# KentaYoshii/Raymarcher

Measured on AMD Instinct MI355X. Metric: Mpixels/s at 3840x2160 Mandelbulb, 256 march steps, higher is better.
Workload: dtype f32

## Files before the change

raymarcher_amd/csrc/rm_device.hip.h:

```cpp
#pragma once
#include "../../include/raymarcher_amd.h"
#include <type_traits>

#include "rm_math.hip.h"
#include "rm_internal.h"

namespace rm {

struct V3 { float x, y, z; };
struct V4 { float x, y, z, w; };

RM_DEV V3 v3(float x, float y, float z) { return V3{x, y, z}; }
RM_DEV V4 v4(float x, float y, float z, float w) { return V4{x, y, z, w}; }
RM_DEV V3 add(V3 a, V3 b) { return v3(a.x + b.x, a.y + b.y, a.z + b.z); }
RM_DEV V3 sub(V3 a, V3 b) { return v3(a.x - b.x, a.y - b.y, a.z - b.z); }
RM_DEV V3 mul(V3 a, V3 b) { return v3(a.x * b.x, a.y * b.y, a.z * b.z); }
RM_DEV V3 scale(V3 a, float s) { return v3(a.x * s, a.y * s, a.z * s); }
RM_DEV V3 neg(V3 a) { return v3(-a.x, -a.y, -a.z); }
RM_DEV V3 madd(V3 a, float s, V3 b) { return v3(fma(a.x, s, b.x), fma(a.y, s, b.y), fma(a.z, s, b.z)); }
RM_DEV float dot2(float ax, float ay, float bx, float by) { return fma(ay, by, ax * bx); }
RM_DEV float dot(V3 a, V3 b) { return fma(a.z, b.z, fma(a.y, b.y, a.x * b.x)); }
RM_DEV float len2(float x, float y) { return sqrt_(dot2(x, y, x, y)); }
RM_DEV float len(V3 a) { return sqrt_(dot(a, a)); }
RM_DEV V3 normalize(V3 a) { float inv = rcp_(len(a)); return scale(a, inv); }
// ... 6 lines not shown
  return (k < 0.0f) ? v3(0.0f, 0.0f, 0.0f) : r;
}
RM_DEV V3 mix(V3 a, V3 b, float t) { return v3(mix_(a.x, b.x, t), mix_(a.y, b.y, t), mix_(a.z, b.z, t)); }

constexpr float kSurfaceDist = 0.001f;

struct Counters { unsigned long long evals, iters, shades, fbm9, fbmd8, shapes; };

}
#include "rm_scene_block.h"
#include "rm_sampler.hip.h"
#include "rm_env.hip.h"
namespace rm {

struct LightSplit { int part; float *slot; int tileIndex; };
struct SceneMin { int idx; float d; V4 trap; };
struct MarchRes { int obj; float d; V4 trap; };
struct Hit { V3 rd, p, n; int obj; };
struct RenderOut { V3 col; int isEnv; float d; };


RM_DEV float sdBox(V3 p, float bx, float by, float bz) {
  float qx = fabs_(p.x) - bx, qy = fabs_(p.y) - by, qz = fabs_(p.z) - bz;
  V3 qm = v3(max_(qx, 0.0f), max_(qy, 0.0f), max_(qz, 0.0f));
  return len(qm) + min_(max_(qx, max_(qy, qz)), 0.0f);
}
RM_DEV float sdCone(V3 p, float r, float h) {
  float pox = len2(p.x, p.z) - r, poy = p.y + h;
  float ex = -r, ey = 2.0f * h;
  float t = clamp_(RM_DIVR_CONST(dot2(pox, poy, ex, ey), dot2(ex, ey, ex, ey)), 0.0f, 1.0f);
  float qx = fma(-ex, t, pox), qy = fma(-ey, t, poy);
  float d = len2(qx, qy);
  return (max_(qx, qy) > 0.0f) ? d : -min_(d, poy);
}
RM_DEV float sdCylinder(V3 p, float h, float r) {
  float dx = len2(p.x, p.z) - r, dy = fabs_(p.y) - h;
  return min_(max_(dx, dy), 0.0f) + len2(max_(dx, 0.0f), max_(dy, 0.0f));
}
RM_DEV float sdOctahedron(V3 p, float s) {
  p = v3(fabs_(p.x), fabs_(p.y), fabs_(p.z));
  float m = ((p.x + p.y) + p.z) - s;
  float rx = fma(3.0f, p.x, -m), ry = fma(3.0f, p.y, -m), rz = fma(3.0f, p.z, -m);
  bool cx = rx < 0.0f, cy = ry < 0.0f, cz = rz < 0.0f;
  V3 q = cx ? p : (cy ? v3(p.y, p.z, p.x) : v3(p.z, p.x, p.y));
  float k = clamp_(0.5f * ((q.z - q.y) + s), 0.0f, s);
  float dl = len(v3(q.x, (q.y - s) + k, q.z - k));
  return (cx || cy || cz) ? dl : (m * 0.57735027f);
}
RM_DEV float sdTorus(V3 p, float tx, float ty) { return len2(len2(p.x, p.z) - tx, p.y) - ty; }
RM_DEV float sdCapsule(V3 p, float h, float r) {
  p.y = p.y - clamp_(p.y, 0.0f, h);
  return len(p) - r;
}
RM_DEV float sdDeathStar(V3 p2, float ra, float rb, float d) {
  float px = p2.x, py = len2(p2.y, p2.z);
  float a = (((ra * ra) - (rb * rb)) + (d * d)) / (2.0f * d);
  float b = sqrt_(max_((ra * ra) - (a * a), 0.0f));
  float inner = len2(px - a, py - b);
  float outer = max_(len2(px, py) - ra, -(len2(px - d, py) - rb));
  return (fma(px, b, -(py * a)) > d * max_(b - py, 0.0f)) ? inner : outer;
}

RM_DEV float sdMandelBrot(const SceneBlock *sb, float px, float py) {
  float ltime = fma(-0.5f, cos_(sb->g.iTime * 0.06f), 0.5f);
  float zoom = pow_(0.9f, 50.0f * ltime);
  float k = (0.045f * zoom) * fma(-ltime, 0.5f, 1.0f);
  float cx = -0.745f - k, cy = 0.186f - k;
  float ld2 = 1.0f;
  float lz2 = dot2(px, py, px, py);
  const int n = sb->s.maxSteps;
  for (int i = 0; i < n; i++) {
    ld2 = ld2 * (4.0f * lz2);
    float nx = fma(px, px, -(py * py)) + cx;
    float ny = fma(2.0f * px, py, cy);
    px = nx; py = ny;
    lz2 = dot2(px, py, px, py);
    if (lz2 > 200.0f) break;
  }
  float d = sqrt_(lz2 / ld2) * log_(lz2);
  return sqrt_(clamp_((150.0f / zoom) * d, 0.0f, 1.0f));
}

enum BulbMode { BULB_GENERIC = 0, BULB_TRIG8 = 1, BULB_ALGEBRAIC8 = 2 };
template <int COUNT, int MODE, bool TRAPMIN, bool TRAP, bool NOJULIA = false>
RM_DEV float bulbIterate(const SceneBlock *sb, V3 pos, V4 &resColor, Counters &cnt) {
  const float power = (MODE == BULB_GENERIC) ? sb->g.power : 8.0f;
  const float pexp = (power - 1.0f) / 2.0f;
  const int iters = sb->s.fractalIters;
  const bool julia = !NOJULIA && len2(sb->g.juliaSeed[0], sb->g.juliaSeed[1]) != 0.0f;
  const bool angleSafe = (MODE != BULB_GENERIC) || fabs_(power) < 1.0e6f;
  const PowPlan planPower = powPlanUniform(power), planPexp = powPlanUniform(pexp);
  V3 w = pos;
  float m = dot(w, w);
  V4 trap = v4(fabs_(w.x), fabs_(w.y), fabs_(w.z), m);
  float dz = 1.0f;
  const V3 c = NOJULIA ? pos : (julia ? v3(sb->g.juliaSeed[0], sb->g.juliaSeed[1], 0.0f) : pos);
  for (int i = 0; i < iters; i++) {
    if (COUNT) cnt.iters++;
    const float mx = absmax_(w.x, w.z);
    const bool raw = (MODE != BULB_ALGEBRAIC8) && __ballot(!(mx >= 3.5527136788e-15f) || !(m < __builtin_inff())) == 0;
    auto step = [&](auto rawTag) __attribute__((always_inline)) {
      constexpr bool RAW = decltype(rawTag)::value;
      float r = RAW ? sqrt_noscale_(m) : sqrt_fast_(m);
      if (MODE == BULB_ALGEBRAIC8) {
        dz = fma(8.0f * (((m * m) * m) * r), dz, 1.0f);
        float rho = sqrt_fast_(dot2(w.x, w.z, w.x, w.z));
        float inv = rcp_(rho);
        float cz = (rho == 0.0f) ? 1.0f : w.z * inv, sx = (rho == 0.0f) ? 0.0f : w.x * inv;
        float re = w.y, im = rho;
#pragma unroll
        for (int k = 0; k < 3; k++) {
          float t = fma(re, re, -(im * im));
          im = 2.0f * (re * im);
          re = t;
          t = fma(cz, cz, -(sx * sx));
          sx = 2.0f * (cz * sx);
          cz = t;
        }
        w = v3(fma(im, sx, c.x), re + c.y, fma(im, cz, c.z));
      } else {
        float pm, pr;
        if (MODE == BULB_TRIG8) {
          pm = (m * (m * m)) * r;
          float r2 = r * r, r4 = r2 * r2;
          pr = r4 * r4;
        } else {
          pm = powApply(m, pexp, planPexp);
          pr = powApply(r, power, planPower);
        }
        dz = fma(power * pm, dz, 1.0f);
        float b = power * acos_(RAW ? w.y * rcp_raw_(r) : divr_(w.y, r));
        float a = power * atan2_mx_<RAW>(w.x, w.z, mx);
        float sb_, cb_, sa_, ca_;
        if (angleSafe) { sincos_inrange_(b, sb_, cb_); sincos_inrange_(a, sa_, ca_); }
        else { sincos_(b, sb_, cb_); sincos_(a, sa_, ca_); }
        w = v3(fma(pr, sb_ * sa_, c.x), fma(pr, cb_, c.y), fma(pr, sb_ * ca_, c.z));
      }
    };
    if (raw) step(std::true_type{}); else step(std::false_type{});
    if (TRAP) {
      if (TRAPMIN) trap = v4(trap.x, hwmin_abs_(trap.y, w.y), hwmin_abs_(trap.z, w.z), hwmin_(trap.w, m));
      else trap = v4(trap.x, min_(trap.y, fabs_(w.y)), min_(trap.z, fabs_(w.z)), min_(trap.w, m));
    }
    m = dot(w, w);
    if (m > 2.0f) break;
  }
  resColor = v4(m, trap.y, trap.z, trap.w);
  return divr_((0.25f * log_(m)) * sqrt_fast_(m), dz);
}
template <int COUNT, bool TRAPMIN, bool TRAP, bool PLAIN = false>
RM_DEV float sdMandelBulb(const SceneBlock *sb, V3 pos, V4 &resColor, Counters &cnt) {
  if (PLAIN || sb->g.power == 8.0f) {
    if (sb->s.features & RM_FEAT_BULB_POWER8_ALGEBRAIC) return bulbIterate<COUNT, BULB_ALGEBRAIC8, TRAPMIN, TRAP, PLAIN>(sb, pos, resColor, cnt);
    return bulbIterate<COUNT, BULB_TRIG8, TRAPMIN, TRAP, PLAIN>(sb, pos, resColor, cnt);
  }
  return bulbIterate<COUNT, BULB_GENERIC, TRAPMIN, TRAP>(sb, pos, resColor, cnt);
}

RM_DEV float sdSierpinski(V3 p) {
  const float Scale = 1.85f, Offset = 2.0f;
  const float k = Offset * (Scale - 1.0f);
  for (int n = 0; n < 14; n++) {
    if (p.x + p.y < 0.0f) { float t = p.x; p.x = -p.y; p.y = -t; }
    if (p.x + p.z < 0.0f) { float t = p.x; p.x = -p.z; p.z = -t; }
    if (p.y + p.z < 0.0f) { float t = p.z; p.z = -p.y; p.y = -t; }
    p = v3(fma(p.x, Scale, -k), fma(p.y, Scale, -k), fma(p.z, Scale, -k));
  }
  return len(p) * pow_(Scale, -14.0f);
}

template <int TRAP, int LEVELS, bool STILL>
RM_DEV float mengerImpl(const SceneBlock *sb, V3 p, V4 &res) {
  float d = sdBox(p, 1.0f, 1.0f, 1.0f);
  float ty = 1.0f, tz = 0.0f;
  const float ani = sb->mengerAni, off = sb->mengerOff;
  const int levels = LEVELS > 0 ? LEVELS : sb->s.mengerLevels;
  const bool still = STILL || ani == 0.0f;
  auto level = [&](int m, float divc, float hs, float sNext) __attribute__((always_inline)) {
    if (!still) {
      V3 v = v3(p.x + off, p.y + off, p.z + off);
      V3 mv = v3(fma(-0.80f, v.z, fma(0.00f, v.y, 0.60f * v.x)), fma(0.00f, v.z, fma(1.00f, v.y, 0.00f * v.x)),
                 fma(0.60f, v.z, fma(0.00f, v.y, 0.80f * v.x)));
      p = mix(p, mv, ani);
    }
    V3 a = v3(fma(2.0f, fract_(p.x * hs), -1.0f), fma(2.0f, fract_(p.y * hs), -1.0f), fma(2.0f, fract_(p.z * hs), -1.0f));
    float rx = fabs_(fma(-3.0f, fabs_(a.x), 1.0f)), ry = fabs_(fma(-3.0f, fabs_(a.y), 1.0f)),
          rz = fabs_(fma(-3.0f, fabs_(a.z), 1.0f));
    float da = 0.0f, db = 0.0f, dc = 0.0f, med;
    if (TRAP == 1) {
      da = __builtin_fmaxf(rx, ry); db = __builtin_fmaxf(ry, rz); dc = __builtin_fmaxf(rz, rx);
      med = __builtin_fminf(da, __builtin_fminf(db, dc));
    } else {
      med = __builtin_amdgcn_fmed3f(rx, ry, rz);
    }
    const float num = med - 1.0f;
    const float c = (divc > 0.0f) ? divc_(num, divc, 1.0f / divc) : (num / sNext);
    const bool up = c > d;
    d = up ? c : d;
    if (TRAP == 1) {
      const float t = __builtin_fminf(ty, ((0.2f * da) * db) * dc);
      ty = up ? t : ty;
    }
    if (TRAP) tz = up ? ((1.0f + (float)m) / 4.0f) : tz;
  };
  if (levels > 0) level(0, 3.0f, 0.5f, 0.0f);
  if (levels > 1) level(1, 9.0f, 1.5f, 0.0f);
  if (levels > 2) level(2, 27.0f, 4.5f, 0.0f);
  if (levels > 3) level(3, 81.0f, 13.5f, 0.0f);
  if (levels > 4) level(4, 243.0f, 40.5f, 0.0f);
  if (levels > 5) level(5, 729.0f, 121.5f, 0.0f);
  if (levels > 6) level(6, 2187.0f, 364.5f, 0.0f);
  if (levels > 7) level(7, 6561.0f, 1093.5f, 0.0f);
  float s = 6561.0f;
  for (int m = 8; m < levels; m++) {
    const float hs = 0.5f * s;
    s = s * 3.0f;
    level(m, 0.0f, hs, s);
  }
  res = v4(d, ty, tz, 0.0f);
  return d;
}
template <int TRAP>
RM_DEV float sdMengerSponge(const SceneBlock *sb, V3 p, V4 &res) {
  const int levels = sb->s.mengerLevels;
  if (sb->mengerAni == 0.0f) {
    if (levels == 5) return mengerImpl<TRAP, 5, true>(sb, p, res);
    if (levels == 4) return mengerImpl<TRAP, 4, true>(sb, p, res);
  }
  return mengerImpl<TRAP, 0, false>(sb, p, res);
}

template <int BULB, int COUNT, int TRAP, bool SKIP, bool TRACK>
RM_DEV SceneMin sdSceneImpl(const SceneBlock *sb, V3 p, Counters &cnt, float ub, float &second) {
  SceneMin res;
  if (TRACK) second = __builtin_inff();
  res.d = 1000000.0f;
  res.idx = -1;
  res.trap = v4(0.0f, 0.0f, 0.0f, 0.0f);
  if (COUNT) cnt.evals++;
  const int n = BULB ? 1 : sb->numObjects;
  for (int i = 0; i < n; i++) {
    const EvalRecord &o = sb->evalRec[i];
    float M[12];
#pragma unroll
    for (int c = 0; c < 4; c++)
      for (int r = 0; r < 3; r++) M[c * 3 + r] = BULB ? sb->objs[0].invModel[c * 4 + r] : o.m[c * 3 + r];
    const float scaleFactor = BULB ? sb->objs[0].scaleFactor : o.scaleFactor;
    auto transform = [&]() __attribute__((always_inline)) {
      return v3(fma(M[6], p.z, fma(M[3], p.y, fma(M[0], p.x, M[9]))),
                fma(M[7], p.z, fma(M[4], p.y, fma(M[1], p.x, M[10]))),
                fma(M[8], p.z, fma(M[5], p.y, fma(M[2], p.x, M[11]))));
    };
    V3 po;
    if (BULB == kBulbPlain) {
      po = p;
      if (__ballot(!(dot(p, p) < __builtin_inff())) != 0ull) po = transform();
    } else {
      po = transform();
    }
    if (SKIP && !BULB) {
      const float lim = fma(ub, o.invScale, o.boundR), pp = dot(po, po);
      const bool far = (lim >= 0.0f) && (pp > (lim * lim) * 1.00003f);
      if (__ballot(!far) == 0ull) {
        if (TRACK) {
          const float v = fma(__builtin_amdgcn_sqrtf(pp), 0.9999f, -o.boundR) * scaleFactor;
          second = min_(second, fma(-fabs_(v), 1.0e-4f, v));
        }
        continue;
      }
    }
    if (COUNT) cnt.shapes++;
    float d;
    const int type = BULB ? (int)RM_MANDELBULB : o.type;
    switch (type) {
      case RM_CUBE: d = sdBox(po, 0.5f, 0.5f, 0.5f); break;
      case RM_CONE: d = sdCone(po, 0.5f, 0.5f); break;
      case RM_CYLINDER: d = sdCylinder(po, 0.5f, 0.5f); break;
      case RM_SPHERE: d = len(po) - 0.5f; break;
      case RM_OCTAHEDRON: d = sdOctahedron(po, 0.5f); break;
      case RM_TORUS: d = sdTorus(po, 0.5f, 0.125f); break;
      case RM_CAPSULE: d = sdCapsule(po, 0.5f, 0.1f); break;
      case RM_DEATHSTAR: d = sdDeathStar(po, 0.5f, 0.35f, 0.5f); break;
      case RM_RECTANGLE: d = sdBox(po, 0.5f, 0.5f, 0.0f); break;
      case RM_MANDELBROT: d = sdMandelBrot(sb, po.x, po.y); break;
      case RM_MANDELBULB: d = sdMandelBulb<COUNT, BULB && COUNT == 0, TRAP != 0, BULB == kBulbPlain>(sb, po, res.trap, cnt); break;
      case RM_MENGERSPONGE: d = sdMengerSponge<TRAP>(sb, po, res.trap); break;
      case RM_SIERPINSKI: d = sdSierpinski(po); break;
      default: continue;
    }
    float cur = (BULB == kBulbPlain) ? d : d * scaleFactor;
    if (TRACK) {
      const float other = (cur < res.d) ? res.d : ((cur >= res.d) ? cur : -__builtin_inff());
      second = min_(second, other);
    }
    if (cur < res.d) { res.d = cur; res.idx = i; }
    if (SKIP && !BULB) ub = min_(ub, cur);
  }
  return res;
}
template <int BULB, int COUNT, int TRAP = 1, bool SKIP = false>
RM_DEV SceneMin sdScene(const SceneBlock *sb, V3 p, Counters &cnt, float ub = __builtin_inff()) {
  float unused;
  return sdSceneImpl<BULB, COUNT, TRAP, SKIP, false>(sb, p, cnt, ub, unused);
}
template <int COUNT>
RM_DEV SceneMin sdSceneOne(const SceneBlock *sb, int j, V3 p, Counters &cnt) {
  SceneMin res;
  res.trap = v4(0.0f, 0.0f, 0.0f, 0.0f);
  res.idx = j;
  if (COUNT) { cnt.evals++; cnt.shapes++; }
  const EvalRecord &o = sb->evalRec[j];
  float M[12];
#pragma unroll
  for (int c = 0; c < 12; c++) M[c] = o.m[c];
  const V3 po = v3(fma(M[6], p.z, fma(M[3], p.y, fma(M[0], p.x, M[9]))),
                   fma(M[7], p.z, fma(M[4], p.y, fma(M[1], p.x, M[10]))),
                   fma(M[8], p.z, fma(M[5], p.y, fma(M[2], p.x, M[11]))));
  float d = 0.0f;
  switch (o.type) {
    case RM_CUBE: d = sdBox(po, 0.5f, 0.5f, 0.5f); break;
    case RM_CONE: d = sdCone(po, 0.5f, 0.5f); break;
    case RM_CYLINDER: d = sdCylinder(po, 0.5f, 0.5f); break;
    case RM_SPHERE: d = len(po) - 0.5f; break;
    case RM_OCTAHEDRON: d = sdOctahedron(po, 0.5f); break;
    case RM_TORUS: d = sdTorus(po, 0.5f, 0.125f); break;
    case RM_CAPSULE: d = sdCapsule(po, 0.5f, 0.1f); break;
    case RM_DEATHSTAR: d = sdDeathStar(po, 0.5f, 0.35f, 0.5f); break;
    default: d = sdBox(po, 0.5f, 0.5f, 0.0f); break;
  }
  res.d = d * o.scaleFactor;
  return res;
}
RM_DEV float nextMinBound(float d, float lipLen, float depth) {
  const float ub = fma(fabs_(d), lipLen, d);
  return fma(fabs_(ub), 1.0e-4f, ub) + fma(depth, 1.0e-6f, 1.0e-5f);
}

template <int BULB, int COUNT, bool SKIP = false>
RM_DEV V3 getNormal(const SceneBlock *sb, V3 p, Counters &cnt, float ub = __builtin_inff()) {
  const float ex = (1.0f * 0.5773f) * 0.0005f, ey = (-1.0f * 0.5773f) * 0.0005f;
  float d[4];
#pragma unroll 1
  for (int k = 0; k < 4; k++) {
    float ox = (k == 0 || k == 3) ? ex : ey;
    float oy = (k >= 2) ? ex : ey;
    float oz = (k == 1 || k == 3) ? ex : ey;
    float v = sdScene<BULB, COUNT, false, SKIP>(sb, v3(p.x + ox, p.y + oy, p.z + oz), cnt, ub).d;
    d[0] = (k == 0) ? v : d[0];
    d[1] = (k == 1) ? v : d[1];
    d[2] = (k == 2) ? v : d[2];
    d[3] = (k == 3) ? v : d[3];
  }
  V3 n;
  n.x = fma(ex, d[3], fma(ey, d[2], fma(ey, d[1], ex * d[0])));
  n.y = fma(ex, d[3], fma(ex, d[2], fma(ey, d[1], ey * d[0])));
  n.z = fma(ex, d[3], fma(ey, d[2], fma(ex, d[1], ey * d[0])));
  return normalize(n);
}

RM_DEV float bulbCullEnd(const SceneBlock *sb, V3 ro, V3 rd, float end) {
  const RmObject &o = sb->objs[0];
  const float jx = sb->g.juliaSeed[0], jy = sb->g.juliaSeed[1];
  const float seed2 = fma(jx, jx, jy * jy);
  const bool ok = (sb->g.power == 8.0f) && (o.scaleFactor >= 0.01f) && (seed2 <= 4.0f);
  if (!ok) return end;
  const bool tight = (o.scaleFactor >= 0.05f) && (seed2 <= 1.2996f);
  const float R2 = tight ? 1.3225f : 4.41f;
  const float *M = o.invModel;
  const V3 po = v3(fma(M[8], ro.z, fma(M[4], ro.y, fma(M[0], ro.x, M[12]))), fma(M[9], ro.z, fma(M[5], ro.y, fma(M[1], ro.x, M[13]))),
                   fma(M[10], ro.z, fma(M[6], ro.y, fma(M[2], ro.x, M[14]))));
  const V3 pd = v3(fma(M[8], rd.z, fma(M[4], rd.y, M[0] * rd.x)), fma(M[9], rd.z, fma(M[5], rd.y, M[1] * rd.x)),
                   fma(M[10], rd.z, fma(M[6], rd.y, M[2] * rd.x)));
  const float a = dot(pd, pd), b = dot(po, pd), c = dot(po, po) - R2;
  const float disc = fma(b, b, -(a * c));
  float tExit = (sqrt_fast_(max_(disc, 0.0f)) - b) / a;
  tExit = fma(tExit, 1.0001f, 1.0e-3f);
  if (c > 0.0f && (b >= 0.0f || disc < 0.0f)) tExit = -1.0f;
  if (!(a > 0.0f)) return end;
  return min_(end, tExit);
}
template <bool HARD = true>
RM_DEV float sceneCullEnd(const SceneBlock *sb, V3 ro, V3 rd, float end, float R2) {
  if (!sb->cullOk || !(R2 > 0.0f)) return end;
  const V3 po = v3(ro.x - sb->cullC[0], ro.y - sb->cullC[1], ro.z - sb->cullC[2]);
  const float a = dot(rd, rd), b = dot(po, rd), c = dot(po, po) - R2;
  const float disc = fma(b, b, -(a * c));
  float tExit = (sqrt_fast_(max_(disc, 0.0f)) - b) / a;
  tExit = fma(tExit, 1.0001f, 1.0e-3f);
  if (c > 0.0f && (b >= 0.0f || disc < 0.0f)) tExit = -1.0f;
  if (!(a > 0.0f)) return end;
  if (HARD && sb->cullBoxOk) {
    const float tx = ((rd.x >= 0.0f ? sb->cullHi[0] : sb->cullLo[0]) - ro.x) * __builtin_amdgcn_rcpf(rd.x);
    const float ty = ((rd.y >= 0.0f ? sb->cullHi[1] : sb->cullLo[1]) - ro.y) * __builtin_amdgcn_rcpf(rd.y);
    const float tz = ((rd.z >= 0.0f ? sb->cullHi[2] : sb->cullLo[2]) - ro.z) * __builtin_amdgcn_rcpf(rd.z);
    const float tb = min_(min_(tx, ty), tz);
    tExit = min_(tExit, fma(fabs_(tb), 1.0e-4f, tb) + 1.0e-3f);
  }
  return min_(end, tExit);
}
template <int BULB, int COUNT, bool SHADOW, bool CULL = false>
RM_DEV MarchRes march(const SceneBlock *sb, V3 ro, V3 rd, float end, float side, Counters &cnt, float ub0 = __builtin_inff()) {
  if (CULL && COUNT != 1) {
    const bool softRay = SHADOW && sb->s.enableSoftShadow != 0;
    if (BULB && !softRay) end = bulbCullEnd(sb, ro, rd, end);
    else if (softRay) end = sceneCullEnd<false>(sb, ro, rd, end, sb->cullR2Soft);
    else end = sceneCullEnd<true>(sb, ro, rd, end, sb->cullR2);
  }
  float depth = 0.0f;
  float pen = 1.0f;
  SceneMin c;
  c.d = 1000000.0f; c.idx = -1; c.trap = v4(0.0f, 0.0f, 0.0f, 0.0f);
  const int steps = sb->s.maxSteps;
  const bool soft = SHADOW && sb->s.enableSoftShadow != 0;
  constexpr bool SKIP = CULL && !BULB && COUNT != 1;
  const float lipLen = SKIP ? (sb->cullLip * len(rd)) * 1.0001f : 0.0f;
  float ub = ub0;
  float second = -__builtin_inff();
  for (int i = 0; i < steps; i++) {
    const V3 p = madd(rd, depth, ro);
    bool one = false;
    int nearU = 0;
    if (SKIP) {
      nearU = __builtin_amdgcn_readfirstlane(c.idx);
      one = sb->cullOneOk && __ballot(!(c.idx == nearU && nearU >= 0 && second > ub)) == 0ull;
    }
    if (SKIP && one) c = sdSceneOne<COUNT>(sb, nearU, p, cnt);
    else c = sdSceneImpl<BULB, COUNT, !SHADOW, SKIP, SKIP>(sb, p, cnt, ub, second);
    if (fabs_(c.d) < kSurfaceDist || depth > end) break;
    if (SHADOW) {
      if (soft) pen = min_(pen, divr_(8.0f * c.d, depth));
      depth = depth + fabs_(c.d);
    } else {
      depth = fma(c.d, side, depth);
    }
    if (SKIP) {
      ub = nextMinBound(c.d, lipLen, depth);
      second = fma(fabs_(c.d), -(lipLen * 1.0001f), second) - fma(depth, 1.0e-6f, 1.0e-5f);
    }
  }
  MarchRes r;
  bool hit = fabs_(c.d) < kSurfaceDist;
  r.obj = hit ? c.idx : -1;
  r.trap = c.trap;
  if (SHADOW) r.d = pen;
  else r.d = hit ? (depth - c.d) : depth;
  return r;
}

RM_DEV float permute(float x) {
  const float y = fma(x, 34.0f, 1.0f) * x;
  return fma(-289.0f, floor_(RM_DIVC(y, 289.0f)), y);
}
RM_DEV float taylorInvSqrt(float r) { return fma(-0.85373472095314f, r, 1.79284291400159f); }
RM_DEV float fade(float t) { return ((t * t) * t) * fma(t, fma(t, 6.0f, -15.0f), 10.0f); }

RM_DEV void pgrad(float ixyz, float &gx, float &gy, float &gz) {
  float x = RM_DIVC(ixyz, 7.0f);
  float y = fract_(RM_DIVC(floor_(x), 7.0f)) - 0.5f;
  x = fract_(x);
  float z = (0.5f - fabs_(x)) - fabs_(y);
  float sz = step_(z, 0.0f);
  gx = fma(-sz, step_(0.0f, x) - 0.5f, x);
  gy = fma(-sz, step_(0.0f, y) - 0.5f, y);
  gz = z;
}
RM_DEV float pcorner(float ixyz, float fx, float fy, float fz) {
  float gx, gy, gz;
  pgrad(ixyz, gx, gy, gz);
  V3 g = v3(gx, gy, gz);
  g = scale(g, taylorInvSqrt(dot(g, g)));
  return dot(g, v3(fx, fy, fz));
}
RM_DEV float pnoise(V3 p) {
  float i0x = floor_(p.x), i0y = floor_(p.y), i0z = floor_(p.z);
  float i1x = mod_(i0x + 1.0f, 256.0f), i1y = mod_(i0y + 1.0f, 256.0f), i1z = mod_(i0z + 1.0f, 256.0f);
  i0x = mod_(i0x, 256.0f); i0y = mod_(i0y, 256.0f); i0z = mod_(i0z, 256.0f);
  float f0x = fract_(p.x), f0y = fract_(p.y), f0z = fract_(p.z);
  float f1x = f0x - 1.0f, f1y = f0y - 1.0f, f1z = f0z - 1.0f;
  float px0 = permute(i0x), px1 = permute(i1x);
  float ixy00 = permute(px0 + i0y), ixy10 = permute(px1 + i0y);
  float ixy01 = permute(px0 + i1y), ixy11 = permute(px1 + i1y);
  float n000 = pcorner(permute(ixy00 + i0z), f0x, f0y, f0z);
  float n100 = pcorner(permute(ixy10 + i0z), f1x, f0y, f0z);
  float n010 = pcorner(permute(ixy01 + i0z), f0x, f1y, f0z);
  float n110 = pcorner(permute(ixy11 + i0z), f1x, f1y, f0z);
  float n001 = pcorner(permute(ixy00 + i1z), f0x, f0y, f1z);
  float n101 = pcorner(permute(ixy10 + i1z), f1x, f0y, f1z);
  float n011 = pcorner(permute(ixy01 + i1z), f0x, f1y, f1z);
  float n111 = pcorner(permute(ixy11 + i1z), f1x, f1y, f1z);
  float fx = fade(f0x), fy = fade(f0y), fz = fade(f0z);
  float nzx = mix_(n000, n001, fz), nzy = mix_(n100, n101, fz), nzz = mix_(n010, n011, fz), nzw = mix_(n110, n111, fz);
  float nyx = mix_(nzx, nzz, fy), nyy = mix_(nzy, nzw, fy);
  return 2.2f * mix_(nyx, nyy, fx);
}
RM_DEV V3 bumpNormal(V3 normal, V3 pos) {
  V3 ps = scale(pos, 10.0f);
  float nv = pnoise(ps);
  float g[3];
#pragma unroll 1
  for (int k = 0; k < 3; k++) {
// ... 247 lines not shown
  const int nl = sb->numLights;
  const bool soft = sb->s.enableSoftShadow != 0;
  if (BULB && !RES && COUNT != 1) {
    if (hardDirectionalOnly(sb)) {
      uint32_t need = 0u;
      for (int i = 0; i < nl; i++) {
        const RmLight &li = sb->lights[i];
        const V3 L = normalize(v3(-li.dir[0], -li.dir[1], -li.dir[2]));
        if (!(dot(N, L) <= 0.005f)) need |= 1u << i;
      }
      const uint32_t hitMask = shadowQueue<BULB, COUNT, CULLS>(sb, so, need, far, cnt);
      return hardLightSum(sb, mat, N, p, V, far, ks, hitMask, total);
    }
  }
  for (int i = 0; i < nl; i++) {
    const RmLight &li = sb->lights[i];
    if (RES && li.type == RM_LIGHT_AREA) {
      V3 p1 = v3(li.points[0][0], li.points[0][1], li.points[0][2]);
      V3 side1 = sub(v3(li.points[1][0], li.points[1][1], li.points[1][2]), p1);
      V3 side2 = sub(v3(li.points[3][0], li.points[3][1], li.points[3][2]), p1);
      V3 toL = sub(madd(side2, rd.y + 0.0f, madd(side1, rd.x + 0.0f, p1)), p);
      V3 L = normalize(toL);
      if (dot(N, L) <= 0.005f) continue;
      MarchRes sh = march<BULB, COUNT, true, CULLS>(sb, so, L, len(toL), 1.0f, cnt, ubSo);
      if (sh.obj != -1 && objs[sh.obj].lightIdx != i) continue;
      total = add(total, getAreaLight(sb, N, V, p, li, mat));
      continue;
    }
    LightGeom g = lightSetup(li, p, far);
    MarchRes sh;
    sh.obj = -1; sh.d = 1.0f; sh.trap = v4(0.0f, 0.0f, 0.0f, 0.0f);
    const bool need = COUNT == 1 || !(dot(N, g.L) <= 0.005f);
    if (partial) {
      if (i == split.part && need) {
        sh = march<BULB, COUNT, true, CULLS>(sb, so, g.L, g.maxT, 1.0f, cnt, ubSo);
        split.slot[2 * i] = __int_as_float(sh.obj);
        split.slot[2 * i + 1] = sh.d;
      }
      continue;
    }
    if (need) {
      if (SPLIT == 2) { sh.obj = __float_as_int(split.slot[2 * i]); sh.d = split.slot[2 * i + 1]; }
      else sh = march<BULB, COUNT, true, CULLS>(sb, so, g.L, g.maxT, 1.0f, cnt, ubSo);
    }
    V3 cur;
    if (lightTerm(li, g, mat, N, V, ks, sh.obj, sh.d, soft, cur)) total = add(total, cur);
  }
  return total;
}

RM_DEV V3 bulbTrapColor(float ty, float tz, float tw) {
  V3 c = v3(0.2f, 0.2f, 0.2f);
  c = mix(c, v3(0.10f, 0.20f, 0.30f), clamp_(ty, 0.0f, 1.0f));
  c = mix(c, v3(0.02f, 0.10f, 0.30f), clamp_(tz * tz, 0.0f, 1.0f));
  c = mix(c, v3(0.30f, 0.10f, 0.02f), clamp_(pow_(tw, 6.0f), 0.0f, 1.0f));
  return scale(c, 0.5f);
}

constexpr int kPoolWaves = 4, kPoolList = 64 * RM_MAX_LIGHTS;
static_assert(RM_MAX_LIGHTS <= 16, "a pool entry holds the light in 10 bits, a hit mask 16 lights");
template <int BULB, int COUNT>
RM_DEV uint32_t shadowPool(const SceneBlock *sb, V3 so, uint32_t pend, float dStart, float far, Counters &cnt) {
  __shared__ uint16_t s_list[kPoolWaves][kPoolList];
  __shared__ uint32_t s_hits[kPoolWaves][32];
  const int wave = (int)(threadIdx.x >> 6), lane = (int)__lane_id();
  uint16_t *list = s_list[wave];
  uint32_t *hitw = s_hits[wave];
  hitw[lane >> 1] = 0u;
  const int nl = sb->numLights;
  uint32_t n = 0u;
  for (int i = 0; i < nl; i++) {
    const bool mine = ((pend >> i) & 1u) != 0u;
    const uint64_t m = __ballot(mine);
    const uint32_t rank = __builtin_amdgcn_mbcnt_hi((uint32_t)(m >> 32), __builtin_amdgcn_mbcnt_lo((uint32_t)m, 0u));
    if (mine) list[n + rank] = (uint16_t)(lane | (i << 6));
    n += (uint32_t)__popcll(m);
  }
  __builtin_amdgcn_wave_barrier();
  const int maxSteps = sb->s.maxSteps;
  int cur = -1, own = 0, step = 0;
  V3 o = so, L = v3(0.0f, 0.0f, 0.0f);
  float depth = 0.0f, end = 0.0f;
  uint32_t next = 0u;
  for (;;) {
    const uint64_t idle = __ballot(cur < 0);
    if (idle != 0ull && next < n) {
      const uint32_t k = next + __builtin_amdgcn_mbcnt_hi((uint32_t)(idle >> 32), __builtin_amdgcn_mbcnt_lo((uint32_t)idle, 0u));
      next += (uint32_t)__popcll(idle);
      const bool take = cur < 0 && k < n;
      uint32_t e = 0u;
      if (take) e = list[k];
      const int src = (int)(e & 63u);
      const V3 os = v3(__shfl(so.x, src), __shfl(so.y, src), __shfl(so.z, src));
      const float ds = __shfl(dStart, src);
      if (take) {
        cur = (int)(e >> 6);
        own = src;
        o = os;
        const RmLight &li = sb->lights[cur];
        L = normalize(v3(-li.dir[0], -li.dir[1], -li.dir[2]));
        end = bulbCullEnd(sb, o, L, far);
        const bool resume = !(ds < 0.0f);
        depth = resume ? ds : 0.0f;
        step = resume ? 1 : 0;
        if (resume && 0.0f > end) cur = -1;
      }
    }
    if (cur >= 0) {
      const SceneMin c = sdScene<BULB, COUNT, false>(sb, madd(L, depth, o), cnt);
      const bool hit = fabs_(c.d) < kSurfaceDist;
      bool fin = hit || depth > end;
      if (!fin) {
        depth = depth + fabs_(c.d);
        step++;
        fin = step >= maxSteps;
      }
      if (fin) {
        if (hit) atomicOr(&hitw[own >> 1], 1u << (((own & 1) << 4) + cur));
        cur = -1;
      }
    }
    if (__ballot(cur >= 0) == 0ull && next >= n) break;
  }
  __builtin_amdgcn_wave_barrier();
  return (hitw[lane >> 1] >> ((lane & 1) << 4)) & 0xffffu;
}

template <int BULB, int COUNT>
RM_DEV RenderOut renderPooled(const SceneBlock *sb, const RmObject *objs, V3 ro, V3 rd, const MarchRes &res, Hit &info,
                              float maxT, V3 bg, Counters &cnt) {
  const bool surf = res.obj != -1;
  const int nl = sb->numLights;
  V3 p = v3(0.0f, 0.0f, 0.0f), N = p, so = p;
  float ao = 1.0f, dStart = -1.0f;
  uint32_t pend = 0u, hits = 0u;
  if (surf) {
    if (COUNT) cnt.shades++;
    p = madd(rd, res.d, ro);
    N = getNormal<BULB, COUNT>(sb, p, cnt);
    if (sb->s.features & RM_FEAT_PERLIN_BUMP) N = bumpNormal(N, p);
    if (sb->s.enableAmbientOcclusion) ao = calcAO<BULB, COUNT>(sb, p, N, cnt);
    so = shadowOrigin(p, N);
    bool shared = f2u(so.x) != 0x80000000u && f2u(so.y) != 0x80000000u && f2u(so.z) != 0x80000000u;
    uint32_t need = 0u;
    for (int i = 0; i < nl; i++) {
      const RmLight &li = sb->lights[i];
      const V3 L = normalize(v3(-li.dir[0], -li.dir[1], -li.dir[2]));
      shared = shared && (fabs_(L.x) + fabs_(L.y) + fabs_(L.z) <= 2.0f);
      if (!(dot(N, L) <= 0.005f)) need |= 1u << i;
    }
    const int maxSteps = sb->s.maxSteps;
    if (need != 0u && maxSteps > 0) {
      if (!shared) {
        pend = need;
      } else {
        const float d0 = fabs_(sdScene<BULB, COUNT, false>(sb, so, cnt).d);
        if (d0 < kSurfaceDist) hits = need;
        else if (maxSteps > 1) { pend = need; dStart = d0; }
      }
    }
  }
  const uint32_t hitMask = hits | shadowPool<BULB, COUNT>(sb, so, pend, dStart, maxT, cnt);
  RenderOut out;
  if (!surf) {
    out.col = bg;
    out.isEnv = 1;
    out.d = maxT;
    return out;
  }
  out.isEnv = 0;
  out.d = res.d;
  const RmObject &o = objs[0];
  Material mat;
  mat.amb = v3(o.cAmbient[0], o.cAmbient[1], o.cAmbient[2]);
  mat.dif = getDiffuse<false>(sb, o, p);
  mat.spec = v3(o.cSpecular[0], o.cSpecular[1], o.cSpecular[2]);
  mat.shininess = o.shininess;
  const float ka = sb->g.ka, ks = sb->g.ks;
  const V3 total = v3((mat.amb.x * ka) * ao, (mat.amb.y * ka) * ao, (mat.amb.z * ka) * ao);
  const V3 ph = hardLightSum(sb, mat, N, v3(0.0f, 0.0f, 0.0f), normalize(neg(rd)), maxT, ks, hitMask, total);
  const V3 c = bulbTrapColor(res.trap.y, res.trap.z, res.trap.w);
  out.col = v3(c.x * (ph.x * 8.0f), c.y * (ph.y * 8.0f), c.z * (ph.z * 8.0f));
  info.p = p; info.n = N; info.rd = rd; info.obj = res.obj;
  return out;
}

template <int BULB, int COUNT, bool TEX, bool CULLS, int SPLIT = 0, bool POOL = false>
RM_DEV RenderOut render(const SceneBlock *sb, const RmObject *objs, V3 ro, V3 rd, Hit &info, float side, float maxT,
                        V3 bg, Counters &cnt, LightSplit split = LightSplit{-1, nullptr, 0}) {
  RenderOut out;
  info.obj = -1;
  MarchRes res;
  if (SPLIT == 2) {
    const float *q = split.slot + 2 * sb->numLights;
    res.obj = __float_as_int(q[0]); res.d = q[1]; res.trap = v4(q[2], q[3], q[4], q[5]);
  } else {
    res = march<BULB, COUNT, false, CULLS>(sb, ro, rd, maxT, side, cnt);
    if (SPLIT == 1 && split.part == 0) {
// ... 196 lines not shown
```

raymarcher_amd/csrc/rm_math.hip.h:

```cpp
#pragma once
#include <hip/hip_runtime.h>
#include <stdint.h>

namespace rm {

#define RM_DEV __device__ __forceinline__

RM_DEV float fma(float a, float b, float c) { return __builtin_fmaf(a, b, c); }
RM_DEV uint32_t f2u(float f) { return __builtin_bit_cast(uint32_t, f); }
RM_DEV float u2f(uint32_t u) { return __builtin_bit_cast(float, u); }
RM_DEV float fabs_(float x) { return __builtin_fabsf(x); }
RM_DEV float min_(float x, float y) { float r; asm("v_min_f32 %0, %1, %2" : "=v"(r) : "v"(x), "v"(y)); return r; }
RM_DEV float max_(float x, float y) { float r; asm("v_max_f32 %0, %1, %2" : "=v"(r) : "v"(x), "v"(y)); return r; }
RM_DEV float clamp_(float x, float lo, float hi) { return min_(max_(x, lo), hi); }
RM_DEV float floor_(float x) { return __builtin_floorf(x); }
RM_DEV float fract_(float x) { return __builtin_amdgcn_fractf(x); }
RM_DEV float mod_(float x, float y) { return fma(-y, __builtin_floorf(x / y), x); }
RM_DEV float step_(float edge, float x) { return (x < edge) ? 0.0f : 1.0f; }
RM_DEV float mix_(float x, float y, float a) { return fma(y, a, x * (1.0f - a)); }
RM_DEV float sqrt_(float x) { return __builtin_sqrtf(x); }
RM_DEV float rcp_(float y) {
  const float ay = fabs_(y);
  if (__builtin_expect(__ballot(!(ay >= 1.17549435e-38f) || !(ay < 8.50705917e37f)) != 0, 0)) return 1.0f / y;
  const float r = __builtin_amdgcn_rcpf(y);
// ... 83 lines not shown

RM_DEV float asin_p(float z) {
  float p = fma(z, 4.277068377e-02f, 2.384351753e-02f);
  p = fma(z, p, 4.553402960e-02f);
  p = fma(z, p, 7.494829595e-02f);
  p = fma(z, p, 1.666676253e-01f);
  return p;
}
RM_DEV float acos_(float x) {
  float ax;
  asm("v_min_f32 %0, 1.0, |%1|" : "=v"(ax) : "v"(x));
  float p = fma(ax, -1.253449009e-03f, 6.638590246e-03f);
  p = fma(ax, p, -1.704506390e-02f);
  p = fma(ax, p, 3.086272627e-02f);
  p = fma(ax, p, -5.016417801e-02f);
  p = fma(ax, p, 8.897730708e-02f);
  p = fma(ax, p, -2.145987004e-01f);
  p = fma(ax, p, 1.570796251e+00f);
  float v = sqrt_noscale_(1.0f - ax) * p;
  return (x > 0.0f) ? v : (kPi - v);
}

RM_DEV float asin_(float x) {
  float ax = fabs_(x);
  bool small = ax <= 0.5f;
  float z = small ? (x * x) : ((1.0f - ax) * 0.5f);
  float s = small ? x : sqrt_(z);
  float as = fma(s * z, asin_p(z), s);
  float big = kPio2 - 2.0f * as;
  big = (x < 0.0f) ? -big : big;
  float r = small ? as : big;
  float edge = (x > 0.0f) ? kPio2 : -kPio2;
  return (small || ax < 1.0f) ? r : edge;
}

RM_DEV float atan_p(float s) {
  float p = fma(s, 2.920665313e-03f, -1.636782475e-02f);
  p = fma(s, p, 4.321170226e-02f);
  p = fma(s, p, -7.552202046e-02f);
  p = fma(s, p, 1.066599935e-01f);
  p = fma(s, p, -1.421105415e-01f);
  p = fma(s, p, 1.999377310e-01f);
  p = fma(s, p, -3.333315253e-01f);
  return p;
}
template <bool RAW = false>
RM_DEV float atan2_mx_(float y, float x, float mx) {
  float ax = fabs_(x), ay = fabs_(y);
  float mn;
  asm("v_min_f32 %0, |%1|, |%2|" : "=v"(mn) : "v"(x), "v"(y));
  float t = RAW ? mn * rcp_raw_(mx) : divr_(mn, mx);
  t = hwmin1_(t);
  if (!RAW) t = (mx == 0.0f) ? 0.0f : t;
  float s = t * t;
  float a = fma(t * s, atan_p(s), t);
  a = (ay > ax) ? (kPio2 - a) : a;
  a = (x < 0.0f) ? (kPi - a) : a;
  return u2f((f2u(a) & 0x7fffffffu) | (f2u(y) & 0x80000000u));
}
RM_DEV float absmax_(float x, float y) {
  float mx;
  asm("v_max_f32 %0, |%1|, |%2|" : "=v"(mx) : "v"(x), "v"(y));
  return mx;
}
template <bool RAW = false>
RM_DEV float atan2_(float y, float x) { return atan2_mx_<RAW>(y, x, absmax_(x, y)); }

RM_DEV float log2_(float x) {
  uint32_t ux = f2u(x) - 0x3f3504f3u;
  int32_t e = (int32_t)ux >> 23;
  float m = u2f((ux & 0x007fffffu) + 0x3f3504f3u);
  float f = m - 1.0f;
  float l = fma(f, 1.258333027e-01f, -2.072679251e-01f);
  l = fma(f, l, 2.157161385e-01f);
  l = fma(f, l, -2.389451116e-01f);
  l = fma(f, l, 2.879162133e-01f);
  l = fma(f, l, -3.607036769e-01f);
  l = fma(f, l, 4.809106290e-01f);
  l = fma(f, l, -7.213473320e-01f);
  l = fma(f, l, 1.442695022e+00f);
  float r = fma(f, l, (float)e);
  return (x >= 1.17549435e-38f) ? r : -__builtin_inff();
}
RM_DEV float exp2_(float x) {
  float n = __builtin_rintf(x);
  float f = x - n;
  float p = fma(f, 1.535335905e-04f, 1.339887502e-03f);
  p = fma(f, p, 9.618436918e-03f);
  p = fma(f, p, 5.550332367e-02f);
  p = fma(f, p, 2.402264774e-01f);
  p = fma(f, p, 6.931471825e-01f);
  p = fma(f, p, 1.0f);
  uint32_t scale = (f2u(n + 12582912.0f) << 23) + 0x3f800000u;
  float r = p * u2f(scale);
  r = (x >= 128.0f) ? __builtin_inff() : r;
  return (x > -125.0f) ? r : 0.0f;
}
struct PowPlan { int n; bool fast, half, neg; };
RM_DEV PowPlan powPlan(float y) {
  float ay = fabs_(y), two = ay + ay;
  PowPlan pl;
  pl.fast = (two <= 256.0f) && (two == floor_(two));
  pl.n = pl.fast ? (int)ay : 0;
  pl.half = ay != (float)pl.n;
  pl.neg = y < 0.0f;
  return pl;
}
RM_DEV PowPlan powPlanUniform(float y) {
  PowPlan pl = powPlan(y);
  pl.n = __builtin_amdgcn_readfirstlane(pl.n);
  pl.fast = __builtin_amdgcn_readfirstlane((int)pl.fast) != 0;
  pl.half = __builtin_amdgcn_readfirstlane((int)pl.half) != 0;
  pl.neg = __builtin_amdgcn_readfirstlane((int)pl.neg) != 0;
  return pl;
}
RM_DEV float powApply(float x, float y, const PowPlan &pl) {
  if (pl.fast) {
    float p = 1.0f, b = x;
    for (int e = pl.n; e != 0; e >>= 1) {
      if (e & 1) p = p * b;
      if (e > 1) b = b * b;
    }
    if (pl.half) p = p * sqrt_fast_(x);
    return pl.neg ? rcp_(p) : p;
  }
  return exp2_(y * log2_(x));
}
RM_DEV float pow_(float x, float y) { return powApply(x, y, powPlan(y)); }
constexpr float kLn2 = 0.693147182f;
constexpr float kLog2e = 1.44269502f;
RM_DEV float log_(float x) { return log2_(x) * kLn2; }
RM_DEV float exp_(float x) { return exp2_(x * kLog2e); }

}
```

Baseline: 4524.

## Fuse bulb distance epilogue and drop per-step end checks when cull exit is owned

Adds a wave-uniform fast path for the Mandelbulb distance epilogue that uses an unguarded log2 polynomial, a no-scale sqrt and a raw reciprocal when m and dz are known to be in normal range. bulbCullEnd now also reports whether the bounding-sphere exit really bounds the ray. The primary and shadow march loops use this to test the end distance before the SDF evaluation, or only after a step, so a sample past the bound is not evaluated. This trims guard instructions and wasted SDF calls in the hot loop, at the cost of more code variants and extra ballots.

```diff
diff --git a/raymarcher_amd/csrc/rm_device.hip.h b/raymarcher_amd/csrc/rm_device.hip.h
--- a/raymarcher_amd/csrc/rm_device.hip.h
+++ b/raymarcher_amd/csrc/rm_device.hip.h
@@ -112,7 +112,7 @@
 }
 
 enum BulbMode { BULB_GENERIC = 0, BULB_TRIG8 = 1, BULB_ALGEBRAIC8 = 2 };
-template <int COUNT, int MODE, bool TRAPMIN, bool TRAP, bool NOJULIA = false>
+template <int COUNT, int MODE, bool TRAPMIN, bool TRAP, bool NOJULIA = false, bool FUSE = false>
 RM_DEV float bulbIterate(const SceneBlock *sb, V3 pos, V4 &resColor, Counters &cnt) {
   const float power = (MODE == BULB_GENERIC) ? sb->g.power : 8.0f;
   const float pexp = (power - 1.0f) / 2.0f;
@@ -176,13 +176,16 @@
     if (m > 2.0f) break;
   }
   resColor = v4(m, trap.y, trap.z, trap.w);
+  static_assert(!FUSE || MODE != BULB_GENERIC, "the generic power's dz has no known sign: it keeps the guarded forms");
+  if (FUSE && __ballot(!(m >= 1.262177448e-29f) || !(dz < 8.50705917e37f)) == 0ull)
+    return ((0.25f * (log2_raw_(m) * kLn2)) * sqrt_noscale_(m)) * rcp_raw_(dz);
   return divr_((0.25f * log_(m)) * sqrt_fast_(m), dz);
 }
-template <int COUNT, bool TRAPMIN, bool TRAP, bool PLAIN = false>
+template <int COUNT, bool TRAPMIN, bool TRAP, bool PLAIN = false, bool FUSE = false>
 RM_DEV float sdMandelBulb(const SceneBlock *sb, V3 pos, V4 &resColor, Counters &cnt) {
   if (PLAIN || sb->g.power == 8.0f) {
-    if (sb->s.features & RM_FEAT_BULB_POWER8_ALGEBRAIC) return bulbIterate<COUNT, BULB_ALGEBRAIC8, TRAPMIN, TRAP, PLAIN>(sb, pos, resColor, cnt);
-    return bulbIterate<COUNT, BULB_TRIG8, TRAPMIN, TRAP, PLAIN>(sb, pos, resColor, cnt);
+    if (sb->s.features & RM_FEAT_BULB_POWER8_ALGEBRAIC) return bulbIterate<COUNT, BULB_ALGEBRAIC8, TRAPMIN, TRAP, PLAIN, FUSE>(sb, pos, resColor, cnt);
+    return bulbIterate<COUNT, BULB_TRIG8, TRAPMIN, TRAP, PLAIN, FUSE>(sb, pos, resColor, cnt);
   }
   return bulbIterate<COUNT, BULB_GENERIC, TRAPMIN, TRAP>(sb, pos, resColor, cnt);
 }
@@ -313,7 +316,7 @@
       case RM_DEATHSTAR: d = sdDeathStar(po, 0.5f, 0.35f, 0.5f); break;
       case RM_RECTANGLE: d = sdBox(po, 0.5f, 0.5f, 0.0f); break;
       case RM_MANDELBROT: d = sdMandelBrot(sb, po.x, po.y); break;
-      case RM_MANDELBULB: d = sdMandelBulb<COUNT, BULB && COUNT == 0, TRAP != 0, BULB == kBulbPlain>(sb, po, res.trap, cnt); break;
+      case RM_MANDELBULB: d = sdMandelBulb<COUNT, BULB && COUNT == 0, TRAP != 0, BULB == kBulbPlain, BULB != 0>(sb, po, res.trap, cnt); break;
       case RM_MENGERSPONGE: d = sdMengerSponge<TRAP>(sb, po, res.trap); break;
       case RM_SIERPINSKI: d = sdSierpinski(po); break;
       default: continue;
@@ -388,7 +391,8 @@
   return normalize(n);
 }
 
-RM_DEV float bulbCullEnd(const SceneBlock *sb, V3 ro, V3 rd, float end) {
+RM_DEV float bulbCullEnd(const SceneBlock *sb, V3 ro, V3 rd, float end, bool &own) {
+  own = false;
   const RmObject &o = sb->objs[0];
   const float jx = sb->g.juliaSeed[0], jy = sb->g.juliaSeed[1];
   const float seed2 = fma(jx, jx, jy * jy);
@@ -407,7 +411,12 @@
   tExit = fma(tExit, 1.0001f, 1.0e-3f);
   if (c > 0.0f && (b >= 0.0f || disc < 0.0f)) tExit = -1.0f;
   if (!(a > 0.0f)) return end;
+  own = (tExit <= end) && (c > 0.0f || tExit > 0.0f);
   return min_(end, tExit);
+}
+RM_DEV float bulbCullEnd(const SceneBlock *sb, V3 ro, V3 rd, float end) {
+  bool own;
+  return bulbCullEnd(sb, ro, rd, end, own);
 }
 template <bool HARD = true>
 RM_DEV float sceneCullEnd(const SceneBlock *sb, V3 ro, V3 rd, float end, float R2) {
@@ -430,9 +439,10 @@
 }
 template <int BULB, int COUNT, bool SHADOW, bool CULL = false>
 RM_DEV MarchRes march(const SceneBlock *sb, V3 ro, V3 rd, float end, float side, Counters &cnt, float ub0 = __builtin_inff()) {
+  bool own = false;
   if (CULL && COUNT != 1) {
     const bool softRay = SHADOW && sb->s.enableSoftShadow != 0;
-    if (BULB && !softRay) end = bulbCullEnd(sb, ro, rd, end);
+    if (BULB && !softRay) end = bulbCullEnd(sb, ro, rd, end, own);
     else if (softRay) end = sceneCullEnd<false>(sb, ro, rd, end, sb->cullR2Soft);
     else end = sceneCullEnd<true>(sb, ro, rd, end, sb->cullR2);
   }
@@ -446,6 +456,25 @@
   const float lipLen = SKIP ? (sb->cullLip * len(rd)) * 1.0001f : 0.0f;
   float ub = ub0;
   float second = -__builtin_inff();
+  if constexpr (BULB != 0 && CULL && COUNT != 1) {
+    static_assert(!SKIP, "the bulb classes have no single-object fast path");
+    auto bulbLoop = [&](auto preTag) __attribute__((always_inline)) {
+      constexpr bool PRE = decltype(preTag)::value;
+      for (int i = 0; i < steps; i++) {
+        if (PRE && depth > end) break;
+        c = sdSceneImpl<BULB, COUNT, !SHADOW, false, false>(sb, madd(rd, depth, ro), cnt, ub, second);
+        if (fabs_(c.d) < kSurfaceDist || (!PRE && depth > end)) break;
+        if (SHADOW) {
+          if (soft) pen = min_(pen, divr_(8.0f * c.d, depth));
+          depth = depth + fabs_(c.d);
+        } else {
+          depth = fma(c.d, side, depth);
+        }
+      }
+    };
+    if (__ballot(!own) == 0ull) bulbLoop(std::true_type{});
+    else bulbLoop(std::false_type{});
+  } else
   for (int i = 0; i < steps; i++) {
     const V3 p = madd(rd, depth, ro);
     bool one = false;
@@ -859,6 +888,7 @@
   V3 o = so, L = v3(0.0f, 0.0f, 0.0f);
   float depth = 0.0f, end = 0.0f;
   uint32_t next = 0u;
+  bool pre = true;
   for (;;) {
     const uint64_t idle = __ballot(cur < 0);
     if (idle != 0ull && next < n) {
@@ -870,27 +900,39 @@
       const int src = (int)(e & 63u);
       const V3 os = v3(__shfl(so.x, src), __shfl(so.y, src), __shfl(so.z, src));
       const float ds = __shfl(dStart, src);
+      bool endOwn = true;
       if (take) {
         cur = (int)(e >> 6);
         own = src;
         o = os;
         const RmLight &li = sb->lights[cur];
         L = normalize(v3(-li.dir[0], -li.dir[1], -li.dir[2]));
-        end = bulbCullEnd(sb, o, L, far);
+        end = bulbCullEnd(sb, o, L, far, endOwn);
         const bool resume = !(ds < 0.0f);
         depth = resume ? ds : 0.0f;
         step = resume ? 1 : 0;
-        if (resume && 0.0f > end) cur = -1;
+        if ((resume && 0.0f > end) || (endOwn && depth > end)) cur = -1;
       }
+      pre = pre && __ballot(!endOwn) == 0ull;
     }
     if (cur >= 0) {
       const SceneMin c = sdScene<BULB, COUNT, false>(sb, madd(L, depth, o), cnt);
       const bool hit = fabs_(c.d) < kSurfaceDist;
-      bool fin = hit || depth > end;
-      if (!fin) {
-        depth = depth + fabs_(c.d);
-        step++;
-        fin = step >= maxSteps;
+      bool fin;
+      if (pre) {
+        fin = hit;
+        if (!fin) {
+          depth = depth + fabs_(c.d);
+          step++;
+          fin = step >= maxSteps || depth > end;
+        }
+      } else {
+        fin = hit || depth > end;
+        if (!fin) {
+          depth = depth + fabs_(c.d);
+          step++;
+          fin = step >= maxSteps;
+        }
       }
       if (fin) {
         if (hit) atomicOr(&hitw[own >> 1], 1u << (((own & 1) << 4) + cur));
diff --git a/raymarcher_amd/csrc/rm_math.hip.h b/raymarcher_amd/csrc/rm_math.hip.h
--- a/raymarcher_amd/csrc/rm_math.hip.h
+++ b/raymarcher_amd/csrc/rm_math.hip.h
@@ -189,6 +189,21 @@
   float r = fma(f, l, (float)e);
   return (x >= 1.17549435e-38f) ? r : -__builtin_inff();
 }
+RM_DEV float log2_raw_(float x) {
+  uint32_t ux = f2u(x) - 0x3f3504f3u;
+  int32_t e = (int32_t)ux >> 23;
+  float m = u2f((ux & 0x007fffffu) + 0x3f3504f3u);
+  float f = m - 1.0f;
+  float l = fma(f, 1.258333027e-01f, -2.072679251e-01f);
+  l = fma(f, l, 2.157161385e-01f);
+  l = fma(f, l, -2.389451116e-01f);
+  l = fma(f, l, 2.879162133e-01f);
+  l = fma(f, l, -3.607036769e-01f);
+  l = fma(f, l, 4.809106290e-01f);
+  l = fma(f, l, -7.213473320e-01f);
+  l = fma(f, l, 1.442695022e+00f);
+  return fma(f, l, (float)e);
+}
 RM_DEV float exp2_(float x) {
   float n = __builtin_rintf(x);
   float f = x - n;
```

New measurement: 4645, median of 6. 1.03x the previous value.
